# injun-baek/Video-Depth-Normal-v2

Measured on AMD Instinct MI355X. Metric: depth frames/sec at 518x518, ViT-L, higher is better.
Workload: dtype f16x3; 1 GPU; DepthAnythingV2(vitl) batch=8 518x518 streams/GPU, memory bank full (S=6); replicas per GPU; lanes=2, precision=f16x3, ranks=1, backend=none, attention_pv_products=1

## Files before the change

### include/vdn.h

```cpp
#ifndef VDN_H
#define VDN_H
#include <stddef.h>
#include <stdint.h>

#ifdef __cplusplus
extern "C" {
#endif

typedef void* vdn_stream;

enum vdn_status { VDN_OK = 0, VDN_EINVAL = -1, VDN_EUNSUPPORTED = -2, VDN_EALIGN = -3 };
enum vdn_dtype { VDN_F16 = 0, VDN_BF16 = 1, VDN_F32 = 2, VDN_NONE = 3 };
enum vdn_act { VDN_ACT_NONE = 0, VDN_ACT_GELU = 1, VDN_ACT_RELU = 2,
               VDN_ACT_SILU = 3  };
enum vdn_amode { VDN_A_PLAIN = 0, VDN_A_CONV3X3 = 1 };
enum vdn_store {
  VDN_ST_PLAIN = 0,
  VDN_ST_HEADS = 1,
  VDN_ST_CONVT = 2,
  VDN_ST_GEGLU = 3
};

typedef struct vdn_gemm_tuning {
  int force_bm;
// ... 65 lines not shown
  const float* subpix_bias;
} vdn_gemm_desc;

int vdn_gemm(const vdn_gemm_desc* d, vdn_stream stream);

int vdn_layernorm(const void* x, int x_dt, int rows, int C, const float* w, const float* b, float eps,
                  const float* addvec, float alpha, const float* addtab, int tab_div, int tab_mod,
                  int out_group, void* out_h, void* out_h_lo, int h_dt, float* out_f, void* out8, int kt,
                  vdn_stream stream);

int vdn_flash_attn(int dt, const void* Q, const void* K, const void* Vt, void* out, const void* Q_lo,
                   const void* K_lo, const void* Vt_lo, void* out_lo, const void* Q8, const void* K8, void* out8, int out_kt,
                   int B, int H, int nq, int nq_pad, int nk, int nk_pad, float scale, int pv_products, vdn_stream stream);

int vdn_temporal_attn(int dt, const void* qkv, void* out, const void* qkv_lo, void* out_lo, int Bv, int T, int D,
                      int c, int heads, float scale, const float* rope_cs, vdn_stream stream);

int vdn_groupnorm(int dt, const void* x, const void* x_lo, void* y, void* y_lo, int F, int HW, int C, int groups,
                  const float* w, const float* b, float eps, float* partial, int nsplit, vdn_stream stream);

int vdn_upsample_bilinear(int dt, const void* x, const void* x_lo, void* y, void* y_lo, int B, int IH, int IW, int OH,
                          int OW, int C, vdn_stream stream);
int vdn_upsample_bilinear_f32(const float* x, float* y, int B, int IH, int IW, int OH, int OW, int relu,
                              vdn_stream stream);

int vdn_patchify(int dt, const float* img, void* rows, void* rows_lo, int B, int H, int W, int ldk,
                 vdn_stream stream);

int vdn_fill_row(float* x, const float* vec, int B, int rows_per_b, int row, int C, vdn_stream stream);

int vdn_bicubic(const float* src, float* dst, int ih, int iw, int oh, int ow, int C, float scale_rows,
                float scale_cols, vdn_stream stream);

int vdn_preprocess(const uint8_t* frames, int n, int h, int w, int swap_rb, float* out, int H, int W, const float* mean3,
                   const float* std3, vdn_stream stream);

int vdn_add_vec(const float* x, const float* vec, float alpha, float* y, int rows, int C, vdn_stream stream);

int vdn_head_out(int dt, const void* feat, const void* feat_lo, const float* w, float bias, float* depth, int M,
                 int C, int relu, vdn_stream stream);

enum { VDN_OUT_NONE = 0, VDN_OUT_RELU = 1, VDN_OUT_SIGMOID = 2 };

int vdn_head_out_act(int dt, const void* feat, const void* feat_lo, const float* w, float bias, float* depth, int M,
                     int C, int act, float out_scale, vdn_stream stream);

int vdn_mask_down1(const float* depth, float* out, int B, int H, int W, int OH, int OW, const float* w,
                   vdn_stream stream);
int vdn_mask_down2(const float* in, float* out, int B, int H, int W, int OH, int OW, const float* w,
                   vdn_stream stream);

int vdn_dwconv7(const float* x, float* y, int B, int H, int W, int C, const float* w, const float* bias,
                vdn_stream stream);

int vdn_addtab_cast(int dt, const float* x, const float* tab, int tab_div, int tab_mod, void* y, void* y_lo,
                    size_t rows, int C, vdn_stream stream);

int vdn_temporal_attn_last(int dt, const float* pool, size_t slot_stride, const int32_t* slots, int T, int HW, int c,
                           const float* pe_q, const float* pe_k, const float* pe_v, float scale, void* out, void* out_lo,
                           vdn_stream stream);

size_t vdn_stitch_workspace_bytes(void);
int vdn_stitch_fit(const float* pred, const float* target, size_t n, void* workspace, float* coef, vdn_stream stream);
int vdn_stitch_apply(const float* window, const float* coef, float* out_tail, float* out_new, float* ref1, size_t hw,
                     int T, int align_len, int overlap, int ref_frame, vdn_stream stream);

enum vdn_eval_domain { VDN_EVAL_DEPTH = 0, VDN_EVAL_DISP = 1 };
enum vdn_eval_tgm { VDN_EVAL_TGM_ROWS = 0, VDN_EVAL_TGM_FRAMES = 1 };
size_t vdn_eval_workspace_bytes(int frames);
int vdn_eval_fit(const float* pred, const float* gt, const uint8_t* mask, int frames, size_t hw, double dmin, double dmax,
                 int domain, void* workspace, double* coef, vdn_stream stream);
int vdn_eval_metrics(const float* pred, const float* gt, const uint8_t* mask, int frames, int H, int W, double dmin,
                     double dmax, int domain, int tgm, const double* coef, void* workspace, double* out,
                     vdn_stream stream);
int vdn_resize_bilinear_hp(const float* x, float* y, int frames, int IH, int IW, int OH, int OW, vdn_stream stream);

size_t vdn_normal_eval_workspace_bytes(int frames);
int vdn_sobel_ix_iy(const float* depth, float* ix, float* iy, int frames, int H, int W, int normalize_kernel,
                    vdn_stream stream);
int vdn_normal_vector(const float* depth, float* out, int frames, int H, int W, int normalize_kernel, float scale_xy,
                      float scale_z, float eps, vdn_stream stream);
int vdn_erode_mask3(const uint8_t* mask, uint8_t* out, int frames, int H, int W, vdn_stream stream);
int vdn_normal_eval(const float* pred, const float* target, int target_is_depth, const uint8_t* mask, int frames, int H,
                    int W, void* workspace, double* frame_sums, int64_t* frame_counts, double* out, vdn_stream stream);

int vdn_normal_loss_backward_trip(int wide);
int vdn_normal_loss_backward(const float* pred, const float* target, int target_is_depth, const uint8_t* mask, int frames,
                             int H, int W, const double* count, const double* coeff, float* grad_pred, vdn_stream stream);

size_t vdn_depth_loss_workspace_bytes(int B, int T);
int vdn_depth_loss(const float* prediction, const float* target, const uint8_t* mask, int B, int T, int H, int W,
                   double alpha, int scales, double stable_scale, void* workspace, float* scale_shift,
                   double* frame_stats, int64_t* frame_counts, double* out, vdn_stream stream);

size_t vdn_depth_loss_backward_workspace_bytes(int B, int T, int H, int W);
int vdn_depth_loss_backward(const float* prediction, const float* target, const uint8_t* mask, int B, int T, int H, int W,
                            double alpha, int scales, double stable_scale, const float* scale_shift,
                            const double* frame_stats, const int64_t* frame_counts, const double* out, const float* coeff,
                            void* workspace, float* grad_prediction, vdn_stream stream);

size_t vdn_depth_loss_trimmed_workspace_bytes(int B, int T);
int vdn_depth_loss_trimmed(const float* prediction, const float* target, const uint8_t* mask, int B, int T, int H, int W,
                           double alpha, int scales, double stable_scale, double keep, void* workspace, float* scale_shift,
                           double* frame_stats, int64_t* frame_counts, double* out, vdn_stream stream);
size_t vdn_depth_loss_trimmed_backward_workspace_bytes(int B, int T, int H, int W);
int vdn_depth_loss_trimmed_backward(const float* prediction, const float* target, const uint8_t* mask, int B, int T, int H, int W,
// ... 88 lines not shown
```

### video-depth-normal-v2_amd/csrc/spatial.hip

```cpp
#include "common.hpp"
#include "resample.hpp"
#include <stddef.h>

namespace {

template <int DT>
__global__ __launch_bounds__(256) void upsample_kernel(const typename Half<DT>::T* __restrict__ x,
                                                       const typename Half<DT>::T* __restrict__ xl,
                                                       typename Half<DT>::T* __restrict__ y,
                                                       typename Half<DT>::T* __restrict__ yl, int B, int IH, int IW,
                                                       int OH, int OW, int C) {
  using T = typename Half<DT>::T;
  using V8 = typename Half<DT>::V8;
  const int cv = C >> 3;
  const size_t total = (size_t)B * OH * OW * cv;
  const float sy = ac_scale(IH, OH), sx = ac_scale(IW, OW);
  for (size_t i = blockIdx.x * (size_t)256 + threadIdx.x; i < total; i += (size_t)gridDim.x * 256) {
    const int c8 = (int)(i % cv);
    size_t pix = i / cv;
    const int ox = (int)(pix % OW);
    pix /= OW;
    const int oy = (int)(pix % OH);
    const int b = (int)(pix / OH);
    const auto [y0, y1, ly] = ac_coord<AcWeight::rounded>(oy, sy, IH);
// ... 252 lines not shown
                                                      const float* __restrict__ bias, int WT) {
  extern __shared__ __attribute__((aligned(16))) char smem[];
  float* sw = (float*)smem;
  float* sx = sw + 49 * DW_CB;
  const int cblocks = C / DW_CB, rtiles = (H + DW_TH - 1) / DW_TH, ctiles = (W + WT - 1) / WT;
  int bid = blockIdx.x;
  const int cb = (bid % cblocks) * DW_CB;
  bid /= cblocks;
  const int x0 = (bid % ctiles) * WT;
  bid /= ctiles;
  const int oy0 = (bid % rtiles) * DW_TH, b = bid / rtiles;
  const int Wt = (W - x0) < WT ? (W - x0) : WT;
  const int WP = WT + 6;
  for (int i = threadIdx.x; i < 49 * (DW_CB / 4); i += 256) {
    const int t = i / (DW_CB / 4), v = i - t * (DW_CB / 4);
    *(f32x4*)(sw + t * DW_CB + v * 4) = *(const f32x4*)(w + (size_t)t * C + cb + v * 4);
  }
  for (int i = threadIdx.x; i < (DW_TH + 6) * WP * (DW_CB / 4); i += 256) {
    const int v = i % (DW_CB / 4);
    const int p = i / (DW_CB / 4);
    const int r = p / WP, cx = p - r * WP;
    const int iy = oy0 - 3 + r, ix = x0 + cx - 3;
    f32x4 val = {0.f, 0.f, 0.f, 0.f};
    if (iy >= 0 && iy < H && ix >= 0 && ix < W) val = *(const f32x4*)(x + (((size_t)b * H + iy) * W + ix) * C + cb + v * 4);
    *(f32x4*)(sx + (size_t)(r * WP + cx) * DW_PS + v * 4) = val;
  }
  __syncthreads();
  const int v = threadIdx.x & 7, pl = threadIdx.x >> 3;
  const int runs_per_row = (Wt + 3) / 4;
  const f32x4 bv = *(const f32x4*)(bias + cb + v * 4);
  for (int run = pl; run < DW_TH * runs_per_row; run += 32) {
    const int ry = run / runs_per_row, ox0 = (run - ry * runs_per_row) * 4;
    if (oy0 + ry >= H) break;
    f32x4 acc[4] = {bv, bv, bv, bv};
#pragma unroll
    for (int ky = 0; ky < 7; ++ky) {
      const float* row = sx + (size_t)((ry + ky) * WP + ox0) * DW_PS + v * 4;
      f32x4 in[10], wk[7];
#pragma unroll
      for (int i = 0; i < 10; ++i) in[i] = (ox0 + i < WP) ? *(const f32x4*)(row + i * DW_PS) : f32x4{0.f, 0.f, 0.f, 0.f};
#pragma unroll
      for (int kx = 0; kx < 7; ++kx) wk[kx] = *(const f32x4*)(sw + (ky * 7 + kx) * DW_CB + v * 4);
#pragma unroll
      for (int o = 0; o < 4; ++o)
#pragma unroll
        for (int kx = 0; kx < 7; ++kx) acc[o] += in[o + kx] * wk[kx];
    }
#pragma unroll
    for (int o = 0; o < 4; ++o)
      if (ox0 + o < Wt) *(f32x4*)(y + (((size_t)b * H + oy0 + ry) * W + x0 + ox0 + o) * C + cb + v * 4) = acc[o];
  }
}

constexpr int OC_T = 16, OC_NT = 512;
template <int CS>
__global__ __launch_bounds__(OC_NT) void oc1_combine_kernel(const float* __restrict__ z, const float* __restrict__ bias,
                                                          float* __restrict__ out, int IH, int IW, int OH, int OW, int Co,
                                                          int max_pix) {
  extern __shared__ __attribute__((aligned(16))) char smem[];
  float* sz = (float*)smem;
  constexpr int V = CS / 4;
  const float sy = ac_scale(IH, OH), sx = ac_scale(IW, OW);
  const int slices = Co / CS, txn = (OW + OC_T - 1) / OC_T, tyn = (OH + OC_T - 1) / OC_T;
  int bid = blockIdx.x;
  const int cs = (bid % slices) * CS;
  bid /= slices;
  const int ox0 = (bid % txn) * OC_T;
  bid /= txn;
  const int oy0 = (bid % tyn) * OC_T, b = bid / tyn;
  const int ylast = oy0 + OC_T < OH - 1 ? oy0 + OC_T : OH - 1, xlast = ox0 + OC_T < OW - 1 ? ox0 + OC_T : OW - 1;
  constexpr AcWeight R = AcWeight::rounded;
  const int py0 = ac_coord<R>(oy0 > 0 ? oy0 - 1 : 0, sy, IH).i0, px0 = ac_coord<R>(ox0 > 0 ? ox0 - 1 : 0, sx, IW).i0;
  const int py1 = ac_coord<R>(ylast, sy, IH).i1, px1 = ac_coord<R>(xlast, sx, IW).i1;
  const int nph = py1 - py0 + 1, npw = px1 - px0 + 1;
  if (nph * npw > max_pix) return;
  const float* zb = z + ((size_t)b * IH * IW) * 9 * Co + cs;
  const int total = nph * npw * 9 * V;
  constexpr int U = 9;
  for (int base = threadIdx.x; base < total; base += OC_NT * U) {
    f32x4 r[U];
#pragma unroll
    for (int u = 0; u < U; ++u) {
      const int i = base + u * OC_NT;
      if (i < total) {
        const int v = i % V, t = (i / V) % 9, p = i / (9 * V);
        const int pr = p / npw, pc = p - pr * npw;
        r[u] = *(const f32x4*)(zb + ((size_t)(py0 + pr) * IW + px0 + pc) * 9 * Co + t * Co + v * 4);
      }
    }
#pragma unroll
    for (int u = 0; u < U; ++u) {
      const int i = base + u * OC_NT;
      if (i < total) *(f32x4*)(sz + (size_t)i * 4) = r[u];
    }
  }
  __syncthreads();
  for (int i = threadIdx.x; i < OC_T * OC_T * V; i += OC_NT) {
    const int v = i % V, pix = i / V;
    const int oy = oy0 + pix / OC_T, ox = ox0 + pix % OC_T;
    if (oy >= OH || ox >= OW) continue;
    int xa[3], xb[3];
    float xl[3];
#pragma unroll
    for (int kx = 0; kx < 3; ++kx) {
      const int xx = ox + kx - 1;
      AcCoord cx = {0, 0, 0.f};
// ... 118 lines not shown
  PrepNorm nm;
  for (int c = 0; c < 3; ++c) {
    if (!(std3[c] > 0.f)) return VDN_EINVAL;
    nm.mean[c] = mean3[c];
    nm.inv_std[c] = 1.0f / std3[c];
  }
  hipLaunchKernelGGL(preprocess_kernel, dim3(grid_for((size_t)n * H * W, 4096)), dim3(256), 0, (hipStream_t)stream, frames, out,
                     n, h, w, H, W, swap_rb, nm);
  VDN_CHECK_LAUNCH();
  return VDN_OK;
}

extern "C" int vdn_head_out_act(int dt, const void* feat, const void* feat_lo, const float* w, float bias, float* depth,
                                int M, int C, int act, float out_scale, vdn_stream stream) {
  if (!feat || !w || !depth || M <= 0 || C <= 0 || C > 64) return VDN_EINVAL;
  if (act != VDN_OUT_NONE && act != VDN_OUT_RELU && act != VDN_OUT_SIGMOID) return VDN_EINVAL;
  if ((C & 7) || ((uintptr_t)feat & 15)) return VDN_EALIGN;
  const unsigned g = grid_for((size_t)M, 8192);
  hipStream_t s = (hipStream_t)stream;
  return with_half(dt, [&](auto t) -> int {
    using T = typename Half<decltype(t)::value>::T;
    hipLaunchKernelGGL(head_out_kernel<decltype(t)::value>, dim3(g), dim3(256), 0, s, (const T*)feat, (const T*)feat_lo, w, bias, depth,
                       M, C, act, out_scale);
    VDN_CHECK_LAUNCH();
    return VDN_OK;
  });
}

extern "C" int vdn_head_out(int dt, const void* feat, const void* feat_lo, const float* w, float bias, float* depth,
                            int M, int C, int relu, vdn_stream stream) {
  return vdn_head_out_act(dt, feat, feat_lo, w, bias, depth, M, C, relu ? VDN_OUT_RELU : VDN_OUT_NONE, 1.f, stream);
}

extern "C" int vdn_mask_down1(const float* depth, float* out, int B, int H, int W, int OH, int OW, const float* w,
                              vdn_stream stream) {
  if (!depth || !out || !w || B <= 0 || OH != (H + 2 - 3) / 2 + 1 || OW != (W + 2 - 3) / 2 + 1) return VDN_EINVAL;
  hipLaunchKernelGGL(mask_down1_kernel, dim3(grid_for((size_t)B * OH * OW, 4096)), dim3(256), 0, (hipStream_t)stream, depth,
                     out, B, H, W, OH, OW, w);
  VDN_CHECK_LAUNCH();
  return VDN_OK;
}

extern "C" int vdn_mask_down2(const float* in, float* out, int B, int H, int W, int OH, int OW, const float* w,
                              vdn_stream stream) {
  if (!in || !out || !w || B <= 0 || OH != (H - 7) / 7 + 1 || OW != (W - 7) / 7 + 1 || OH <= 0 || OW <= 0)
    return VDN_EINVAL;
  const size_t total = (size_t)B * OH * OW;
  hipLaunchKernelGGL(mask_down2_kernel, dim3((unsigned)((total + 127) / 128)), dim3(128), 0, (hipStream_t)stream, in,
                     out, B, H, W, OH, OW, w);
  VDN_CHECK_LAUNCH();
  return VDN_OK;
}

extern "C" int vdn_dwconv7(const float* x, float* y, int B, int H, int W, int C, const float* w, const float* bias,
                           vdn_stream stream) {
  if (!x || !y || !w || !bias || B <= 0 || H <= 0 || W <= 0 || C <= 0) return VDN_EINVAL;
  if (C % DW_CB) return VDN_EALIGN;
  const int WT = ((size_t)49 * DW_CB + (size_t)(DW_TH + 6) * (W + 6) * DW_PS) * sizeof(float) <= 160 * 1024 ? W : 64;
  const size_t lds = ((size_t)49 * DW_CB + (size_t)(DW_TH + 6) * (WT + 6) * DW_PS) * sizeof(float);
  static const hipError_t attr = hipFuncSetAttribute((const void*)dwconv7_kernel, hipFuncAttributeMaxDynamicSharedMemorySize, 160 * 1024);
  if (attr != hipSuccess) return -(1000 + (int)attr);
  hipLaunchKernelGGL(dwconv7_kernel, dim3(B * ((H + DW_TH - 1) / DW_TH) * ((W + WT - 1) / WT) * (C / DW_CB)), dim3(256), lds,
                     (hipStream_t)stream, x, y, B, H, W, C, w, bias, WT);
  VDN_CHECK_LAUNCH();
  return VDN_OK;
}

extern "C" size_t vdn_sizeof_gemm_desc(void) { return sizeof(vdn_gemm_desc); }
extern "C" size_t vdn_offsetof_gemm_zeros(void) { return offsetof(vdn_gemm_desc, zeros); }
extern "C" size_t vdn_offsetof_gemm_res2_lo(void) { return offsetof(vdn_gemm_desc, res2_lo); }

extern "C" const char* vdn_version(void) { return "vdn-hip 0.1 (gfx950)"; }

extern "C" int vdn_arch_ok(void) {
  hipDeviceProp_t prop;
  if (hipGetDeviceProperties(&prop, 0) != hipSuccess) return 0;
  const char* a = prop.gcnArchName;
  return (a[0] == 'g' && a[1] == 'f' && a[2] == 'x' && a[3] == '9' && a[4] == '5' && a[5] == '0') ? 1 : 0;
}
```

### video-depth-normal-v2_amd/vdn/_abi.py

```python
from __future__ import annotations

import ctypes as C
import os

PKG = os.path.dirname(os.path.dirname(os.path.abspath(__file__)))
LIB_PATH = os.environ.get("VDN_LIB") or os.path.join(PKG, "lib", "libvdn_hip.so")

F16, BF16, F32, NONE = 0, 1, 2, 3
ACT_NONE, ACT_GELU, ACT_RELU, ACT_SILU = 0, 1, 2, 3
OUT_NONE, OUT_RELU, OUT_SIGMOID = 0, 1, 2
A_PLAIN, A_CONV3X3 = 0, 1
ST_PLAIN, ST_HEADS, ST_CONVT, ST_GEGLU = 0, 1, 2, 3
EVAL_DEPTH, EVAL_DISP = 0, 1
EVAL_TGM_ROWS, EVAL_TGM_FRAMES = 0, 1
PACK_LINEAR, PACK_CONV3X3, PACK_CONV3X3_TAPS, PACK_CONVT, PACK_GEGLU, PACK_ROPE = 0, 1, 2, 3, 4, 5

i32, vp, fp = C.c_int32, C.c_void_p, C.c_void_p


class GemmDesc(C.Structure):
    _fields_ = [
        ("dt", i32), ("M", i32), ("N", i32), ("K", i32),
        ("A", vp), ("a_mode", i32), ("lda", i32), ("relu_a", i32),
        ("cB", i32), ("cH", i32), ("cW", i32), ("cC", i32), ("cOH", i32), ("cOW", i32), ("cstride", i32),
# ... 26 lines not shown
class VdnError(RuntimeError):
    pass


def _load():
    if not os.path.exists(LIB_PATH):
        raise ImportError(
            f"{LIB_PATH} not found: the HIP extension is required (there is no CPU fallback). "
            f"Build it with `python __graft_entry__.py build` (hipcc --offload-arch=gfx950).")
    try:
        return C.CDLL(LIB_PATH)
    except OSError as e:
        raise ImportError(f"cannot load {LIB_PATH}: {e}. Rebuild with `python __graft_entry__.py build`.") from e


lib = _load()

EXPORTS = {
    "vdn_gemm": (C.c_int, [C.POINTER(GemmDesc), vp]),
    "vdn_gemm_get_tuning": (C.c_int, [C.POINTER(GemmTuning)]),
    "vdn_layernorm": (C.c_int, [vp, C.c_int, C.c_int, C.c_int, fp, fp, C.c_float, fp, C.c_float, fp, C.c_int, C.c_int,
                                C.c_int, vp, vp, C.c_int, fp, vp, C.c_int, vp]),
    "vdn_flash_attn": (C.c_int, [C.c_int, vp, vp, vp, vp, vp, vp, vp, vp, vp, vp, vp, C.c_int, C.c_int, C.c_int, C.c_int, C.c_int,
                                 C.c_int, C.c_int, C.c_float, C.c_int, vp]),
    "vdn_temporal_attn": (C.c_int, [C.c_int, vp, vp, vp, vp, C.c_int, C.c_int, C.c_int, C.c_int, C.c_int, C.c_float, fp, vp]),
    "vdn_groupnorm": (C.c_int, [C.c_int, vp, vp, vp, vp, C.c_int, C.c_int, C.c_int, C.c_int, fp, fp, C.c_float, fp,
                                C.c_int, vp]),
    "vdn_upsample_bilinear": (C.c_int, [C.c_int, vp, vp, vp, vp, C.c_int, C.c_int, C.c_int, C.c_int, C.c_int, C.c_int, vp]),
    "vdn_upsample_bilinear_f32": (C.c_int, [fp, fp, C.c_int, C.c_int, C.c_int, C.c_int, C.c_int, C.c_int, vp]),
    "vdn_patchify": (C.c_int, [C.c_int, fp, vp, vp, C.c_int, C.c_int, C.c_int, C.c_int, vp]),
    "vdn_fill_row": (C.c_int, [fp, fp, C.c_int, C.c_int, C.c_int, C.c_int, vp]),
    "vdn_bicubic": (C.c_int, [fp, fp, C.c_int, C.c_int, C.c_int, C.c_int, C.c_int, C.c_float, C.c_float, vp]),
    "vdn_preprocess": (C.c_int, [vp, C.c_int, C.c_int, C.c_int, C.c_int, fp, C.c_int, C.c_int, C.POINTER(C.c_float), C.POINTER(C.c_float), vp]),
    "vdn_add_vec": (C.c_int, [fp, fp, C.c_float, fp, C.c_int, C.c_int, vp]),
    "vdn_head_out": (C.c_int, [C.c_int, vp, vp, fp, C.c_float, fp, C.c_int, C.c_int, C.c_int, vp]),
    "vdn_depth_tail": (C.c_int, [C.c_int, fp, C.c_int, C.c_int, C.c_int, C.c_int, vp, vp, C.c_int, fp, fp, C.c_float, fp,
                                 C.c_int, C.c_int, C.c_int, vp]),
    "vdn_head_out_act": (C.c_int, [C.c_int, vp, vp, fp, C.c_float, fp, C.c_int, C.c_int, C.c_int, C.c_float, vp]),
    "vdn_depth_tail_act": (C.c_int, [C.c_int, fp, C.c_int, C.c_int, C.c_int, C.c_int, vp, vp, C.c_int, fp, fp, C.c_float, fp,
                                     C.c_int, C.c_int, C.c_int, C.c_float, vp]),
    "vdn_depth_to_points": (C.c_int, [fp, vp, C.c_int, C.c_int, C.c_double, C.c_double, vp, vp, vp]),
    "vdn_oc1_combine": (C.c_int, [fp, fp, fp, C.c_int, C.c_int, C.c_int, C.c_int, C.c_int, C.c_int, vp]),
    "vdn_pack_rows": (C.c_int, [C.c_int, C.c_int, C.c_int, C.c_int]),
    "vdn_pack_ldb": (C.c_int, [C.c_int, C.c_int, C.c_int, C.c_int]),
    "vdn_pack_weight": (C.c_int, [C.c_int, C.c_int, fp, C.c_int, C.c_int, C.c_int, vp, vp, C.c_int, vp]),
    "vdn_pack_bias": (C.c_int, [C.c_int, fp, C.c_int, C.c_int, C.c_int, fp, vp]),
    "vdn_pack_x8": (C.c_int, [vp, vp, C.c_int, C.c_int, vp, vp, C.c_int, C.c_int, vp]),
    "vdn_pack_x8_f32": (C.c_int, [fp, C.c_int, C.c_int, vp, vp, vp]),
    "vdn_gemm_workspace_bytes": (C.c_size_t, [C.POINTER(GemmDesc)]),
    "vdn_groupnorm_workspace_bytes": (C.c_size_t, [C.c_int, C.c_int, C.c_int]),
    "vdn_mask_down1": (C.c_int, [fp, fp, C.c_int, C.c_int, C.c_int, C.c_int, C.c_int, fp, vp]),
    "vdn_mask_down2": (C.c_int, [fp, fp, C.c_int, C.c_int, C.c_int, C.c_int, C.c_int, fp, vp]),
    "vdn_dwconv7": (C.c_int, [fp, fp, C.c_int, C.c_int, C.c_int, C.c_int, fp, fp, vp]),
    "vdn_addtab_cast": (C.c_int, [C.c_int, fp, fp, C.c_int, C.c_int, vp, vp, C.c_size_t, C.c_int, vp]),
    "vdn_cast": (C.c_int, [vp, C.c_int, vp, C.c_int, C.c_size_t, vp]),
    "vdn_temporal_attn_last": (C.c_int, [C.c_int, fp, C.c_size_t, C.POINTER(C.c_int32), C.c_int, C.c_int, C.c_int, fp, fp, fp,
                                         C.c_float, vp, vp, vp]),
    "vdn_frame_median_workspace_bytes": (C.c_size_t, [C.c_int]),
    "vdn_frame_median": (C.c_int, [fp, C.c_int, C.c_size_t, fp, vp, vp]),
    "vdn_refine_scale": (C.c_int, [fp, fp, C.c_int, C.c_size_t, C.c_float, C.c_float, C.c_float, C.c_float, fp, fp, vp]),
    "vdn_refine_pack": (C.c_int, [fp, fp, C.c_int, C.c_int, C.c_int, C.c_int, vp]),
    "vdn_refine_finish": (C.c_int, [fp, fp, C.c_float, C.c_float, C.c_float, C.c_int, fp, C.c_size_t, vp]),
    "vdn_refine_normalize": (C.c_int, [fp, C.c_float, fp, C.c_size_t, vp]),
    "vdn_refine_mix": (C.c_int, [fp, fp, C.c_float, C.c_float, C.c_float, C.c_float, C.c_float, fp, C.c_size_t, vp]),
    "vdn_dn_attn": (C.c_int, [C.c_int, vp, vp, vp, vp, C.c_int, C.c_int, C.c_int, C.c_int, C.c_int, C.c_int, C.c_int, C.c_int,
                              C.c_int, C.c_float, vp]),
    "vdn_dn_prologue": (C.c_int, [C.c_int, fp, fp, C.c_int, C.c_int, C.c_int, fp, C.c_int, fp, vp, vp, vp]),
    "vdn_dn_tail": (C.c_int, [fp, C.c_int, C.c_int, C.c_int, C.c_int, fp, fp, C.c_int, C.c_int, fp, C.c_int, fp, fp, fp, vp]),
    "vdn_hiera_embed": (C.c_int, [C.c_int, fp, vp, vp, C.c_int, C.c_int, vp]),
    "vdn_hiera_attn": (C.c_int, [C.c_int, vp, vp, vp, vp, C.c_int, C.c_int, C.c_int, C.c_int, C.c_int, C.c_float, vp]),
    "vdn_hiera_pool": (C.c_int, [fp, fp, C.c_int, C.c_int, C.c_int, vp]),
    "vdn_hiera_reroll": (C.c_int, [fp, fp, C.c_int, C.c_int, C.c_int, vp]),
    "vdn_stitch_workspace_bytes": (C.c_size_t, []),
    "vdn_stitch_fit": (C.c_int, [fp, fp, C.c_size_t, vp, fp, vp]),
    "vdn_stitch_apply": (C.c_int, [fp, fp, fp, fp, fp, C.c_size_t, C.c_int, C.c_int, C.c_int, C.c_int, vp]),
    "vdn_eval_workspace_bytes": (C.c_size_t, [C.c_int]),
    "vdn_eval_fit": (C.c_int, [fp, fp, vp, C.c_int, C.c_size_t, C.c_double, C.c_double, C.c_int, vp, vp, vp]),
    "vdn_eval_metrics": (C.c_int, [fp, fp, vp, C.c_int, C.c_int, C.c_int, C.c_double, C.c_double, C.c_int, C.c_int, vp, vp, vp, vp]),
    "vdn_resize_bilinear_hp": (C.c_int, [fp, fp, C.c_int, C.c_int, C.c_int, C.c_int, C.c_int, vp]),
    "vdn_normal_eval_workspace_bytes": (C.c_size_t, [C.c_int]),
    "vdn_sobel_ix_iy": (C.c_int, [fp, fp, fp, C.c_int, C.c_int, C.c_int, C.c_int, vp]),
    "vdn_normal_vector": (C.c_int, [fp, fp, C.c_int, C.c_int, C.c_int, C.c_int, C.c_float, C.c_float, C.c_float, vp]),
    "vdn_erode_mask3": (C.c_int, [vp, vp, C.c_int, C.c_int, C.c_int, vp]),
    "vdn_normal_eval": (C.c_int, [fp, fp, C.c_int, vp, C.c_int, C.c_int, C.c_int, vp, vp, vp, vp, vp]),
    "vdn_normal_loss_backward_trip": (C.c_int, [C.c_int]),
    "vdn_normal_loss_backward": (C.c_int, [fp, fp, C.c_int, vp, C.c_int, C.c_int, C.c_int, vp, vp, fp, vp]),
    "vdn_depth_loss_workspace_bytes": (C.c_size_t, [C.c_int, C.c_int]),
    "vdn_depth_loss": (C.c_int, [fp, fp, vp, C.c_int, C.c_int, C.c_int, C.c_int, C.c_double, C.c_int, C.c_double, vp, fp, vp, vp, vp,
                                 vp]),
    "vdn_depth_loss_backward_workspace_bytes": (C.c_size_t, [C.c_int, C.c_int, C.c_int, C.c_int]),
    "vdn_depth_loss_backward": (C.c_int, [fp, fp, vp, C.c_int, C.c_int, C.c_int, C.c_int, C.c_double, C.c_int, C.c_double, fp, vp, vp, vp,
                                          fp, vp, fp, vp]),
    "vdn_depth_loss_trimmed_workspace_bytes": (C.c_size_t, [C.c_int, C.c_int]),
    "vdn_depth_loss_trimmed": (C.c_int, [fp, fp, vp, C.c_int, C.c_int, C.c_int, C.c_int, C.c_double, C.c_int, C.c_double, C.c_double, vp,
                                         fp, vp, vp, vp, vp]),
    "vdn_depth_loss_trimmed_backward_workspace_bytes": (C.c_size_t, [C.c_int, C.c_int, C.c_int, C.c_int]),
    "vdn_depth_loss_trimmed_backward": (C.c_int, [fp, fp, vp, C.c_int, C.c_int, C.c_int, C.c_int, C.c_double, C.c_int, C.c_double, fp,
                                                  vp, vp, vp, fp, vp, fp, vp]),
    "vdn_prep_trip": (C.c_int, [C.c_int]),
    "vdn_prep_depth_workspace_bytes": (C.c_size_t, [C.c_int]),
    "vdn_prep_rgb": (C.c_int, [fp, fp, C.c_int, C.c_int, C.c_int, C.c_int, vp]),
    "vdn_prep_depth": (C.c_int, [fp, vp, fp, C.c_int, C.c_int64, C.c_int, C.c_int, C.c_int, vp, fp, vp]),
    "vdn_metric_trip": (C.c_int, [C.c_int]),
    "vdn_metric_workspace_bytes": (C.c_size_t, [C.c_int]),
    "vdn_metric_eval": (C.c_int, [fp, fp, vp, C.c_int, C.c_int, C.c_int, C.c_int, C.c_int, C.c_int, C.c_double, C.c_double, vp, vp, vp]),
    "vdn_silog_loss_workspace_bytes": (C.c_size_t, []),
# ... 59 lines not shown
```

### video-depth-normal-v2_amd/vdn/engine.py

```python
from __future__ import annotations

import math
import os
from typing import List, Optional

import torch

from . import _abi as abi
from . import pack
from .runtime import HL, Runtime, ceil_to

GELU, RELU = abi.ACT_GELU, abi.ACT_RELU
PATCH = 14


class EncoderEngine:

    def __init__(self, rt: Runtime, mod, cfg: dict):
        self.rt, self.cfg = rt, cfg
        self.C, self.heads, self.depth, self.taps = cfg["dim"], cfg["heads"], cfg["depth"], cfg["taps"]
        h = rt.prec
        self.w_patch = pack.patch_embed(mod.patch_embed.proj.weight, h)
        self.b_patch = pack.f32(mod.patch_embed.proj.bias)
        self.cls = pack.f32(mod.cls_token).reshape(-1)
# ... 386 lines not shown
        if fused:
            o1 = self._conv3(p1, self.oc1[0], Bf, s0[0], s0[1], F, F // 2, "out1_f32", bias=self.oc1[1], f32_out=True)
            rt.depth_tail(o1, self.oc2_taps, self.oc2[1], self.w_last, self.b_last, depth, Bf, s0[0], s0[1], F // 2, H, W, relu, act, out_scale)
            return depth
        o1 = self._conv3(p1, self.oc1[0], Bf, s0[0], s0[1], F, F // 2, "out1", bias=self.oc1[1])
        up = rt.hbuf("out_up", (Bf * H * W, F // 2))
        rt.upsample(o1, up, Bf, s0[0], s0[1], H, W, F // 2)
        o2 = self._conv3(up, self.oc2[0], Bf, H, W, F // 2, 32, "out2", bias=self.oc2[1], act=RELU)
        rt.head_out(o2, self.w_last, self.b_last, depth, Bf * H * W, 32, relu, act, out_scale)
        return depth


class MemoryEngine:

    def __init__(self, rt: Runtime, mod, C: int, max_len: int):
        self.rt, self.C, self.heads, self.max_len = rt, C, C // 64, max_len
        h = rt.prec
        ma = mod.memory_attention
        self.x8 = rt.x8_capable(C)

        def lin(w, order):
            return pack.Linear(w, order if self.x8 else None)

        NAT, GEMM, ATTN = pack.ORDER_NATURAL, pack.ORDER_GEMM, pack.ORDER_ATTN
        self.layers = []
        for l in ma.layers:
            sa, ca = l.self_attn, l.cross_attn_image
            wqkv, bqkv = pack.cat_proj([sa.q_proj.weight, sa.k_proj.weight, sa.v_proj.weight],
                                       [sa.q_proj.bias, sa.k_proj.bias, sa.v_proj.bias], [1, 1, 0], h)
            wq, bq = pack.cat_proj([ca.q_proj.weight], [ca.q_proj.bias], [1], h)
            wkv, bkv = pack.cat_proj([ca.k_proj.weight, ca.v_proj.weight], [ca.k_proj.bias, ca.v_proj.bias], [1, 0], h)
            self.layers.append(dict(
                n1w=pack.f32(l.norm1.weight), n1b=pack.f32(l.norm1.bias),
                n2w=pack.f32(l.norm2.weight), n2b=pack.f32(l.norm2.bias),
                n3w=pack.f32(l.norm3.weight), n3b=pack.f32(l.norm3.bias),
                wqkv=lin(wqkv, NAT), bqkv=bqkv, wso=lin(pack.linear(sa.out_proj.weight, h), ATTN), bso=pack.f32(sa.out_proj.bias),
                wq=lin(wq, NAT), bq=bq, wkv=lin(wkv, NAT), bkv=bkv,
                wco=lin(pack.linear(ca.out_proj.weight, h), ATTN), bco=pack.f32(ca.out_proj.bias),
                w1=lin(pack.linear(l.linear1.weight, h), NAT), b1=pack.f32(l.linear1.bias),
                w2=lin(pack.linear(l.linear2.weight, h), GEMM), b2=pack.f32(l.linear2.bias)))
        self.nw, self.nb = pack.f32(ma.norm.weight), pack.f32(ma.norm.bias)
        self.curr_pos = pack.f32(mod.curr_pos_enc).reshape(-1)
        self.no_mem = mod.no_mem_embed.detach().float().reshape(1, -1)
        me = mod.memory_encoder

        def flat(*ts):
            return torch.cat([t.detach().float().reshape(-1) for t in ts]).contiguous()

        e0, e1 = me.mask_downsampler[0].encoder, me.mask_downsampler[1].encoder
        self.md1 = flat(e0[0].weight, e0[0].bias, e0[1].weight, e0[1].bias, e0[3].weight, e0[3].bias)
        self.md2 = flat(e1[0].weight, e1[0].bias, e1[1].weight, e1[1].bias, e1[3].weight, e1[3].bias)
        assert self.md1.numel() == 53 and self.md2.numel() == 2598
        self.wpix, self.bpix = pack.conv1x1(me.pix_feat_proj.weight, h), pack.f32(me.pix_feat_proj.bias)
        self.cx = []
        for b in me.fuser.layers:
            self.cx.append(dict(
                wdw=b.dwconv.weight.detach().float().reshape(C, 49).t().contiguous(), bdw=pack.f32(b.dwconv.bias),
                nw=pack.f32(b.norm.weight), nb=pack.f32(b.norm.bias),
                w1=lin(pack.linear(b.pwconv1.weight, h), NAT), b1=pack.f32(b.pwconv1.bias),
                w2=lin(pack.linear(b.pwconv2.weight, h), GEMM), b2=pack.f32(b.pwconv2.bias), g=pack.f32(b.gamma)))
        self.state = {"count": 0, "shape": None}
        self.lane = (0, 1)
        self.bank_rt = rt
        self._rope = {}
        self._nomem = {}

    def clear(self):
        self.state["count"] = 0
        self.state["shape"] = None

    @property
    def S(self):
        return min(self.state["count"], self.max_len)

    def _rope_for(self, side):
        if side not in self._rope:
            self._rope[side] = pack.rope_table(side, side, 64, device=self.rt.device)
        return self._rope[side]

    def prepare(self, B: int, P: int):
        st = self.state
        if st["shape"] != (B, P):
            if st["count"] > 0:
                raise RuntimeError(f"memory bank holds {self.S} frame(s) of batch/grid {st['shape']} but the new frame is "
                                   f"{(B, P)}: call clear_memory() before changing the batch size or resolution")
            st["shape"] = (B, P)
        side = int(math.sqrt(P))
        assert side * side == P, "MemoryBlock assumes square inputs (memory_block.py:85)"
        self._rope_for(side)
        self._bank_full(B, P)

    def commit(self):
        self.state["count"] += 1

    def _bank_full(self, B, P):
        rt, Hh = self.bank_rt, self.heads
        tp = ceil_to(self.max_len * P, 64)
        ks = [rt.hbuf(f"mem_k{l}", (B * Hh, tp, 64), zero=True) for l in range(len(self.layers))]
        vs = [rt.hbuf(f"mem_vt{l}", (B * Hh, 64, tp), zero=True) for l in range(len(self.layers))]
        k8 = [rt.qk8(f"mem_k8{l}", B * Hh, tp) for l in range(len(self.layers))]
        return ks, vs, k8, tp

    def _bank(self, B, P):
        i, n = self.lane
        ks, vs, k8, tp = self._bank_full(B * n, P)
        r0, nr = i * B * self.heads, B * self.heads
# ... 15 lines not shown
        q8, k8 = rt.qk8("ma_q8", B * Hh, pp), rt.qk8("ma_k8", B * Hh, pp)
        ks, vs, k8s, tp = self._bank(B, P)
        S = self.S
        if S == 0:
            nk, nk_pad = P, pp
            if M not in self._nomem:
                self._nomem[M] = rt.to_half(self.no_mem.expand(M, C).contiguous())
            a_nm = self._nomem[M]
            ks = [rt.hbuf(f"nomem_k{l}", (B * Hh, pp, 64), zero=True) for l in range(len(self.layers))]
            vs = [rt.hbuf(f"nomem_vt{l}", (B * Hh, 64, pp), zero=True) for l in range(len(self.layers))]
            k8s = [rt.qk8(f"nomem_k8{l}", B * Hh, pp) for l in range(len(self.layers))]
            for l, L in enumerate(self.layers):
                rt.gemm(a_nm, L["wkv"], M, 2 * C, C, bias=L["bkv"], store=abi.ST_HEADS,
                        heads=rt.head_split([(ks[l], k8s[l])], vs[l], Hh, P, pp, rope_cs=cs, rope_mod=P))
        else:
            nk, nk_pad = S * P, tp
        sh = rt.head_split([(q, q8), (k, k8)], vt, Hh, P, pp, rope_cs=cs, rope_mod=P)
        qh = rt.head_split([(q, q8)], None, Hh, P, pp, rope_cs=cs, rope_mod=P)
        use8 = self.x8 and rt.x8_rows(M) and q8 is not None and rt.pv_products != 3
        n, att, h2 = rt.operand("ma_n", (M, C), use8), rt.operand("ma_att", (M, C), use8), rt.operand("ma_h2", (M, 2 * C), use8)
        for l, L in enumerate(self.layers):
            rt.layernorm(x, M, C, L["n1w"], L["n1b"], 1e-5, out_h=n)
            rt.gemm(n, L["wqkv"], M, 3 * C, C, bias=L["bqkv"], store=abi.ST_HEADS, heads=sh)
            rt.flash_attn(q, k, vt, att, B, Hh, P, pp, P, pp, 0.125, q8=q8, k8=k8)
            rt.gemm(att, L["wso"], M, C, C, bias=L["bso"], res1=x, out=x)
            rt.layernorm(x, M, C, L["n2w"], L["n2b"], 1e-5, out_h=n, addvec=self.curr_pos, alpha=1.0)
            rt.gemm(n, L["wq"], M, C, C, bias=L["bq"], store=abi.ST_HEADS, heads=qh)
            rt.flash_attn(q, ks[l], vs[l], att, B, Hh, P, pp, nk, nk_pad, 0.125, q8=q8, k8=k8s[l])
            rt.gemm(att, L["wco"], M, C, C, bias=L["bco"], res1=x, out=x)
            rt.layernorm(x, M, C, L["n3w"], L["n3b"], 1e-5, out_h=n)
            rt.gemm(n, L["w1"], M, 2 * C, C, bias=L["b1"], act=GELU, out=h2)
            rt.gemm(h2, L["w2"], M, C, 2 * C, bias=L["b2"], res1=x, out=x)
        out = rt.hbuf("mem_out", (M, C))
        rt.layernorm(x, M, C, self.nw, self.nb, 1e-5, out_h=out)
        return out

    def update(self, mem_out: torch.Tensor, depth: torch.Tensor, B: int, ph: int, pw: int):
        rt, C, Hh = self.rt, self.C, self.heads
        P, M = ph * pw, B * ph * pw
        H, W = depth.shape[-2], depth.shape[-1]
        h1, w1 = (H + 2 - 3) // 2 + 1, (W + 2 - 3) // 2 + 1
        h2, w2 = (h1 - 7) // 7 + 1, (w1 - 7) // 7 + 1
        assert (h2, w2) == (ph, pw), "mask downsampler output must match the feature grid (memory_encoder.py:173)"
        m1 = rt.fbuf("me_m1", (B, h1, w1))
        rt.mask_down1(depth, m1, B, H, W, h1, w1, self.md1)
        m2 = rt.fbuf("me_m2", (M,))
        rt.mask_down2(m1, m2, B, h1, w1, h2, w2, self.md2)
        x = rt.fbuf("me_x", (M, C))
        rt.gemm(mem_out, self.wpix, M, C, C, bias=self.bpix, rowadd=m2, out=x)
        d = rt.fbuf("me_dw", (M, C))
        use8 = self.x8 and rt.x8_rows(M)
        n, h4, feat = rt.operand("me_n", (M, C), use8), rt.operand("me_h4", (M, 4 * C), use8), rt.operand("mem_feat", (M, C), use8)
        for cx in self.cx:
            rt.dwconv7(x, d, B, ph, pw, C, cx["wdw"], cx["bdw"])
            rt.layernorm(d, M, C, cx["nw"], cx["nb"], 1e-6, out_h=n)
            rt.gemm(n, cx["w1"], M, 4 * C, C, bias=cx["b1"], act=GELU, out=h4)
            rt.gemm(h4, cx["w2"], M, C, 4 * C, bias=cx["b2"], gamma=cx["g"], res1=x,
                    out=(feat if cx is self.cx[-1] and not use8 else x))
        if use8:
            rt.pack_x8_f32(x, feat.hi, feat.p8)
        ks, vs, k8s, tp = self._bank(B, P)
        slot = self.state["count"] % self.max_len
        cs = self._rope_for(int(math.sqrt(P)))
        for l, L in enumerate(self.layers):
            rt.gemm(feat, L["wkv"], M, 2 * C, C, bias=L["bkv"], store=abi.ST_HEADS,
                    heads=rt.head_split([(ks[l], k8s[l])], vs[l], Hh, P, tp, rope_cs=cs, rope_mod=P, tok_off=slot * P))
```

### video-depth-normal-v2_amd/vdn/runtime.py

```python
from __future__ import annotations

import os

import ctypes as C
from typing import Dict, List, Optional, Sequence, Tuple

import torch

from . import _abi as abi
from ._abi import F16, BF16, F32
from .pack import Linear, Prec

_TDT = {torch.float16: F16, torch.bfloat16: BF16, torch.float32: F32}
_POISON = bool(int(__import__("os").environ.get("VDN_POISON", "0")))


def ceil_to(x: int, m: int) -> int:
    return (x + m - 1) // m * m


class HL:
    __slots__ = ("hi", "lo")

    def __init__(self, hi: torch.Tensor, lo: Optional[torch.Tensor] = None):
# ... 590 lines not shown
        m3, s3 = (C.c_float * 3)(*mean), (C.c_float * 3)(*std)
        self._launch(abi.lib.vdn_preprocess, frames_u8.data_ptr(), n, h, w, int(swap_rb), out.data_ptr(), H, W, m3, s3)
        return out

    def add_vec(self, x, vec, alpha: float, y, rows: int, Cn: int):
        self._launch(abi.lib.vdn_add_vec, x.data_ptr(), vec.data_ptr(), alpha, y.data_ptr(), rows, Cn)

    @staticmethod
    def _out_act(relu: bool, act: Optional[int]) -> int:
        if act is None:
            return abi.OUT_RELU if relu else abi.OUT_NONE
        if act not in (abi.OUT_NONE, abi.OUT_RELU, abi.OUT_SIGMOID):
            raise ValueError(f"act must be one of OUT_NONE, OUT_RELU, OUT_SIGMOID (0, 1, 2), got {act!r}")
        return act

    def depth_tail(self, x: torch.Tensor, w: HL, bias2, w1, b1: float, depth, B: int, IH: int, IW: int, Cn: int, OH: int,
                   OW: int, relu: bool = False, act: Optional[int] = None, out_scale: float = 1.0):
        assert x.dtype == torch.float32 and x.is_contiguous() and w.lo is not None and w.hi.shape[0] == 32
        self._launch(abi.lib.vdn_depth_tail_act, self.dt, x.data_ptr(), B, IH, IW, Cn, w.hi.data_ptr(), w.lo.data_ptr(),
                     w.hi.shape[1], bias2.data_ptr(), w1.data_ptr(), b1, depth.data_ptr(), OH, OW, self._out_act(relu, act),
                     float(out_scale))

    @staticmethod
    def lowres_oc1_rows(M: int) -> bool:
        return M >= int(os.environ.get("VDN_OC1_LOWRES_MIN_ROWS", "65536"))

    def oc1_combine(self, z: torch.Tensor, bias, out: torch.Tensor, B: int, IH: int, IW: int, OH: int, OW: int, Cn: int):
        assert z.dtype == torch.float32 and z.is_contiguous() and z.numel() == B * IH * IW * 9 * Cn, (z.shape, z.dtype)
        assert out.dtype == torch.float32 and out.is_contiguous() and out.numel() == B * OH * OW * Cn, (out.shape, out.dtype)
        self._launch(abi.lib.vdn_oc1_combine, z.data_ptr(), bias.data_ptr(), out.data_ptr(), B, IH, IW, OH, OW, Cn)

    def head_out(self, feat, w, bias: float, depth, M: int, Cn: int, relu: bool = False, act: Optional[int] = None,
                 out_scale: float = 1.0):
        feat, fl = _hl(feat)
        self._launch(abi.lib.vdn_head_out_act, self.dt, feat.data_ptr(), fl, w.data_ptr(), bias, depth.data_ptr(), M, Cn,
                     self._out_act(relu, act), float(out_scale))

    def depth_to_points(self, depth: torch.Tensor, rgb: torch.Tensor, fx: float, fy: float, points: torch.Tensor,
                        colors: torch.Tensor):
        h, w = depth.shape
        assert depth.dtype == torch.float32 and depth.is_contiguous() and rgb.dtype == torch.uint8 and rgb.is_contiguous()
        assert tuple(rgb.shape) == (h, w, 3), (rgb.shape, depth.shape)
        for t in (points, colors):
            assert t.dtype == torch.float64 and t.is_contiguous() and tuple(t.shape) == (h * w, 3), (t.shape, t.dtype)
        self._launch(abi.lib.vdn_depth_to_points, depth.data_ptr(), rgb.data_ptr(), h, w, float(fx), float(fy), points.data_ptr(),
                     colors.data_ptr())

    def mask_down1(self, depth, out, B, H, W, OH, OW, w):
        self._launch(abi.lib.vdn_mask_down1, depth.data_ptr(), out.data_ptr(), B, H, W, OH, OW, w.data_ptr())

    def mask_down2(self, x, out, B, H, W, OH, OW, w):
        self._launch(abi.lib.vdn_mask_down2, x.data_ptr(), out.data_ptr(), B, H, W, OH, OW, w.data_ptr())

    def dwconv7(self, x, y, B, H, W, Cn, w, bias):
        self._launch(abi.lib.vdn_dwconv7, x.data_ptr(), y.data_ptr(), B, H, W, Cn, w.data_ptr(), bias.data_ptr())

    def addtab_cast(self, x, tab, tab_div: int, tab_mod: int, y, rows: int, Cn: int):
        yh, yl = _hl(y)
        self._launch(abi.lib.vdn_addtab_cast, self.dt, x.data_ptr(), self._p(tab), tab_div, tab_mod, yh.data_ptr(), yl, rows, Cn)

    def pack_x8(self, t: HL, hi_kt: torch.Tensor, planes8: torch.Tensor, order: int = 0):
        rows, ld = t.hi.shape
        self._launch(abi.lib.vdn_pack_x8, t.hi.data_ptr(), t.lo.data_ptr(), rows, ld, hi_kt.data_ptr(), planes8.data_ptr(), 1, order)

    def pack_x8_f32(self, x: torch.Tensor, hi_kt: torch.Tensor, planes8: torch.Tensor):
        rows, ld = x.shape
        self._launch(abi.lib.vdn_pack_x8_f32, x.data_ptr(), rows, ld, hi_kt.data_ptr(), planes8.data_ptr())

    def cast(self, x, y):
        self._launch(abi.lib.vdn_cast, x.data_ptr(), _TDT[x.dtype], y.data_ptr(), _TDT[y.dtype], x.numel())
```

Before: 287.1 frames/s.

## Add full-frame-width depthwise 7x7 conv kernel with row-strip LDS tiling

Adds a new depthwise 7x7 convolution kernel for narrow frames (W<=72). Each block stages a whole-width strip of rows for 16 channels in LDS with an odd row stride, then computes runs of 8 output pixels per thread. It becomes the default path, with an environment variable to fall back to the old tiled kernel. The aim is to cut halo reloads and tiling overhead in the memory-encoder fuser's dwconv, at the cost of a different occupancy and LDS footprint.

After: 288.8 frames/s (median of 6 runs). Within noise of the previous version (+0.6%).

```diff
diff --git a/include/vdn.h b/include/vdn.h
--- a/include/vdn.h
+++ b/include/vdn.h
@@ -141,6 +141,10 @@
 
 int vdn_dwconv7(const float* x, float* y, int B, int H, int W, int C, const float* w, const float* bias,
                 vdn_stream stream);
+int vdn_dwconv7_v(const float* x, float* y, int B, int H, int W, int C, const float* w, const float* bias,
+                  int tiled, vdn_stream stream);
+int vdn_dwconv7_plan(int H, int W, int* rows_per_strip, int* row_stride);
+int vdn_dwconv7_task(int W, int rows, int task, int* quad, int* col0, int* row);
 
 int vdn_addtab_cast(int dt, const float* x, const float* tab, int tab_div, int tab_mod, void* y, void* y_lo,
                     size_t rows, int C, vdn_stream stream);
diff --git a/video-depth-normal-v2_amd/csrc/spatial.hip b/video-depth-normal-v2_amd/csrc/spatial.hip
--- a/video-depth-normal-v2_amd/csrc/spatial.hip
+++ b/video-depth-normal-v2_amd/csrc/spatial.hip
@@ -328,6 +328,96 @@
   }
 }
 
+constexpr int DF_CB = 16, DF_NT = 384, DF_RUN = 8, DF_SLACK = 8;
+constexpr size_t DF_LDS_MAX = 76 * 1024;
+
+struct DwFramePlan {
+  int TR, WP;
+  size_t lds;
+};
+inline bool dw_frame_plan(int H, int W, DwFramePlan& p) {
+  if (W > 72) return false;
+  p.WP = (W + 6) | 1;
+  for (int s = 1; s <= H; ++s) {
+    p.TR = (H + s - 1) / s;
+    p.lds = ((size_t)49 * DF_CB + ((size_t)(p.TR + 6) * p.WP + DF_SLACK) * DF_CB) * sizeof(float);
+    if (p.lds <= DF_LDS_MAX) return true;
+  }
+  return false;
+}
+
+struct DwTask { int v, ox0, ry; };
+__host__ __device__ __forceinline__ DwTask dw_frame_task(int task, int rows) {
+  const int t = task >> 2, run = t / rows;
+  return {task & 3, run * DF_RUN, t - run * rows};
+}
+__host__ __device__ __forceinline__ int dw_frame_tasks(int W, int rows) { return ((W + DF_RUN - 1) / DF_RUN) * rows * 4; }
+
+__global__ __launch_bounds__(DF_NT) void dwconv7_frame_kernel(const float* __restrict__ x, float* __restrict__ y, int B, int H,
+                                                             int W, int C, const float* __restrict__ w,
+                                                             const float* __restrict__ bias, int TR, int WP) {
+  extern __shared__ __attribute__((aligned(16))) char smem[];
+  float* sw = (float*)smem;
+  float* sx = sw + 49 * DF_CB;
+  const int cblocks = C / DF_CB, rtiles = (H + TR - 1) / TR;
+  int bid = xcd_remap(blockIdx.x, gridDim.x);
+  const int cb = (bid % cblocks) * DF_CB;
+  bid /= cblocks;
+  const int oy0 = (bid % rtiles) * TR, b = bid / rtiles;
+  if (threadIdx.x < 49 * (DF_CB / 4)) {
+    const int t = threadIdx.x >> 2, v = threadIdx.x & 3;
+    *(f32x4*)(sw + t * DF_CB + v * 4) = *(const f32x4*)(w + (size_t)t * C + cb + v * 4);
+  }
+  const int total = (TR + 6) * WP * (DF_CB / 4);
+  constexpr int U = 6;
+  for (int base = threadIdx.x; base < total; base += DF_NT * U) {
+    f32x4 r[U];
+#pragma unroll
+    for (int u = 0; u < U; ++u) {
+      const int i = base + u * DF_NT;
+      r[u] = f32x4{0.f, 0.f, 0.f, 0.f};
+      if (i < total) {
+        const int v = i & 3, p = i >> 2;
+        const int pr = p / WP, pc = p - pr * WP;
+        const int iy = oy0 - 3 + pr, ix = pc - 3;
+        if (iy >= 0 && iy < H && ix >= 0 && ix < W) r[u] = *(const f32x4*)(x + (((size_t)b * H + iy) * W + ix) * C + cb + v * 4);
+      }
+    }
+#pragma unroll
+    for (int u = 0; u < U; ++u) {
+      const int i = base + u * DF_NT;
+      if (i < total) *(f32x4*)(sx + (size_t)i * 4) = r[u];
+    }
+  }
+  __syncthreads();
+  const int rows = (H - oy0) < TR ? (H - oy0) : TR;
+  const int ntask = dw_frame_tasks(W, rows);
+  for (int task = threadIdx.x; task < ntask; task += DF_NT) {
+    const auto [v, ox0, ry] = dw_frame_task(task, rows);
+    const f32x4 bv = *(const f32x4*)(bias + cb + v * 4);
+    f32x4 acc[DF_RUN];
+#pragma unroll
+    for (int o = 0; o < DF_RUN; ++o) acc[o] = bv;
+#pragma unroll 1
+    for (int ky = 0; ky < 7; ++ky) {
+      const float* row = sx + (size_t)((ry + ky) * WP + ox0) * DF_CB + v * 4;
+      f32x4 in[DF_RUN + 6], wk[7];
+#pragma unroll
+      for (int i = 0; i < DF_RUN + 6; ++i) in[i] = *(const f32x4*)(row + i * DF_CB);
+#pragma unroll
+      for (int kx = 0; kx < 7; ++kx) wk[kx] = *(const f32x4*)(sw + (ky * 7 + kx) * DF_CB + v * 4);
+      __builtin_amdgcn_sched_barrier(0);
+#pragma unroll
+      for (int o = 0; o < DF_RUN; ++o)
+#pragma unroll
+        for (int kx = 0; kx < 7; ++kx) acc[o] += in[o + kx] * wk[kx];
+    }
+#pragma unroll
+    for (int o = 0; o < DF_RUN; ++o)
+      if (ox0 + o < W) *(f32x4*)(y + (((size_t)b * H + oy0 + ry) * W + ox0 + o) * C + cb + v * 4) = acc[o];
+  }
+}
+
 constexpr int OC_T = 16, OC_NT = 512;
 template <int CS>
 __global__ __launch_bounds__(OC_NT) void oc1_combine_kernel(const float* __restrict__ z, const float* __restrict__ bias,
@@ -552,9 +642,36 @@
   return VDN_OK;
 }
 
-extern "C" int vdn_dwconv7(const float* x, float* y, int B, int H, int W, int C, const float* w, const float* bias,
-                           vdn_stream stream) {
+extern "C" int vdn_dwconv7_plan(int H, int W, int* rows_per_strip, int* row_stride) {
+  DwFramePlan p;
+  if (H <= 0 || W <= 0 || !dw_frame_plan(H, W, p)) return 0;
+  if (rows_per_strip) *rows_per_strip = p.TR;
+  if (row_stride) *row_stride = p.WP;
+  return 1;
+}
+
+extern "C" int vdn_dwconv7_task(int W, int rows, int task, int* quad, int* col0, int* row) {
+  if (W <= 0 || rows <= 0 || task < 0 || !quad || !col0 || !row) return -1;
+  const DwTask t = dw_frame_task(task, rows);
+  *quad = t.v, *col0 = t.ox0, *row = t.ry;
+  return dw_frame_tasks(W, rows);
+}
+
+extern "C" int vdn_dwconv7_v(const float* x, float* y, int B, int H, int W, int C, const float* w, const float* bias, int tiled,
+                             vdn_stream stream) {
   if (!x || !y || !w || !bias || B <= 0 || H <= 0 || W <= 0 || C <= 0) return VDN_EINVAL;
+  DwFramePlan p;
+  if (!tiled && dw_frame_plan(H, W, p)) {
+    if ((C % DF_CB) || (((uintptr_t)x | (uintptr_t)y | (uintptr_t)w | (uintptr_t)bias) & 15)) return VDN_EALIGN;
+    const size_t blocks = (size_t)B * ((H + p.TR - 1) / p.TR) * (C / DF_CB);
+    if (blocks >= (1u << 31)) return VDN_EUNSUPPORTED;
+    static const hipError_t attr = hipFuncSetAttribute((const void*)dwconv7_frame_kernel, hipFuncAttributeMaxDynamicSharedMemorySize, (int)DF_LDS_MAX);
+    if (attr != hipSuccess) return -(1000 + (int)attr);
+    hipLaunchKernelGGL(dwconv7_frame_kernel, dim3((unsigned)blocks), dim3(DF_NT), p.lds, (hipStream_t)stream, x, y, B, H, W, C, w, bias,
+                       p.TR, p.WP);
+    VDN_CHECK_LAUNCH();
+    return VDN_OK;
+  }
   if (C % DW_CB) return VDN_EALIGN;
   const int WT = ((size_t)49 * DW_CB + (size_t)(DW_TH + 6) * (W + 6) * DW_PS) * sizeof(float) <= 160 * 1024 ? W : 64;
   const size_t lds = ((size_t)49 * DW_CB + (size_t)(DW_TH + 6) * (WT + 6) * DW_PS) * sizeof(float);
@@ -566,6 +683,11 @@
   return VDN_OK;
 }
 
+extern "C" int vdn_dwconv7(const float* x, float* y, int B, int H, int W, int C, const float* w, const float* bias,
+                           vdn_stream stream) {
+  return vdn_dwconv7_v(x, y, B, H, W, C, w, bias, 0, stream);
+}
+
 extern "C" size_t vdn_sizeof_gemm_desc(void) { return sizeof(vdn_gemm_desc); }
 extern "C" size_t vdn_offsetof_gemm_zeros(void) { return offsetof(vdn_gemm_desc, zeros); }
 extern "C" size_t vdn_offsetof_gemm_res2_lo(void) { return offsetof(vdn_gemm_desc, res2_lo); }
diff --git a/video-depth-normal-v2_amd/vdn/_abi.py b/video-depth-normal-v2_amd/vdn/_abi.py
--- a/video-depth-normal-v2_amd/vdn/_abi.py
+++ b/video-depth-normal-v2_amd/vdn/_abi.py
@@ -102,6 +102,9 @@
     "vdn_mask_down1": (C.c_int, [fp, fp, C.c_int, C.c_int, C.c_int, C.c_int, C.c_int, fp, vp]),
     "vdn_mask_down2": (C.c_int, [fp, fp, C.c_int, C.c_int, C.c_int, C.c_int, C.c_int, fp, vp]),
     "vdn_dwconv7": (C.c_int, [fp, fp, C.c_int, C.c_int, C.c_int, C.c_int, fp, fp, vp]),
+    "vdn_dwconv7_v": (C.c_int, [fp, fp, C.c_int, C.c_int, C.c_int, C.c_int, fp, fp, C.c_int, vp]),
+    "vdn_dwconv7_plan": (C.c_int, [C.c_int, C.c_int, C.POINTER(C.c_int), C.POINTER(C.c_int)]),
+    "vdn_dwconv7_task": (C.c_int, [C.c_int, C.c_int, C.c_int, C.POINTER(C.c_int), C.POINTER(C.c_int), C.POINTER(C.c_int)]),
     "vdn_addtab_cast": (C.c_int, [C.c_int, fp, fp, C.c_int, C.c_int, vp, vp, C.c_size_t, C.c_int, vp]),
     "vdn_cast": (C.c_int, [vp, C.c_int, vp, C.c_int, C.c_size_t, vp]),
     "vdn_temporal_attn_last": (C.c_int, [C.c_int, fp, C.c_size_t, C.POINTER(C.c_int32), C.c_int, C.c_int, C.c_int, fp, fp, fp,
diff --git a/video-depth-normal-v2_amd/vdn/engine.py b/video-depth-normal-v2_amd/vdn/engine.py
--- a/video-depth-normal-v2_amd/vdn/engine.py
+++ b/video-depth-normal-v2_amd/vdn/engine.py
@@ -462,6 +462,7 @@
         self.md2 = flat(e1[0].weight, e1[0].bias, e1[1].weight, e1[1].bias, e1[3].weight, e1[3].bias)
         assert self.md1.numel() == 53 and self.md2.numel() == 2598
         self.wpix, self.bpix = pack.conv1x1(me.pix_feat_proj.weight, h), pack.f32(me.pix_feat_proj.bias)
+        self.dw_tiled = bool(os.environ.get("VDN_DWCONV7_TILED"))
         self.cx = []
         for b in me.fuser.layers:
             self.cx.append(dict(
@@ -583,7 +584,7 @@
         use8 = self.x8 and rt.x8_rows(M)
         n, h4, feat = rt.operand("me_n", (M, C), use8), rt.operand("me_h4", (M, 4 * C), use8), rt.operand("mem_feat", (M, C), use8)
         for cx in self.cx:
-            rt.dwconv7(x, d, B, ph, pw, C, cx["wdw"], cx["bdw"])
+            rt.dwconv7(x, d, B, ph, pw, C, cx["wdw"], cx["bdw"], self.dw_tiled)
             rt.layernorm(d, M, C, cx["nw"], cx["nb"], 1e-6, out_h=n)
             rt.gemm(n, cx["w1"], M, 4 * C, C, bias=cx["b1"], act=GELU, out=h4)
             rt.gemm(h4, cx["w2"], M, C, 4 * C, bias=cx["b2"], gamma=cx["g"], res1=x,
diff --git a/video-depth-normal-v2_amd/vdn/runtime.py b/video-depth-normal-v2_amd/vdn/runtime.py
--- a/video-depth-normal-v2_amd/vdn/runtime.py
+++ b/video-depth-normal-v2_amd/vdn/runtime.py
@@ -666,8 +666,8 @@
     def mask_down2(self, x, out, B, H, W, OH, OW, w):
         self._launch(abi.lib.vdn_mask_down2, x.data_ptr(), out.data_ptr(), B, H, W, OH, OW, w.data_ptr())
 
-    def dwconv7(self, x, y, B, H, W, Cn, w, bias):
-        self._launch(abi.lib.vdn_dwconv7, x.data_ptr(), y.data_ptr(), B, H, W, Cn, w.data_ptr(), bias.data_ptr())
+    def dwconv7(self, x, y, B, H, W, Cn, w, bias, tiled: bool = False):
+        self._launch(abi.lib.vdn_dwconv7_v, x.data_ptr(), y.data_ptr(), B, H, W, Cn, w.data_ptr(), bias.data_ptr(), int(tiled))
 
     def addtab_cast(self, x, tab, tab_div: int, tab_mod: int, y, rows: int, Cn: int):
         yh, yl = _hl(y)
```
